# jkflying/opencalibration

Hardware: AMD Instinct MI355X
Metric: images/sec end-to-end (extract+match+relax) on synthetic aerial grid; LM iters/sec (higher is better)
Workload: dtype f32 (extract) + fp4 0/1 bits, f32 accumulate, exact (match) + f64 (RANSAC, relax)

## Files before the change

### opencalibration_amd/csrc/host/extract_features.cpp

```cpp
#include "../env.hpp"
#include "extract_features.hpp"
#include "sort_like_std.hpp"

#include <algorithm>
#include <cmath>
#include <condition_variable>
#include <cstdio>
#include <cstdlib>
#include <cstring>
#include <deque>
#include <limits>
#include <mutex>
#include <thread>

#include <emmintrin.h>
#include <omp.h>

namespace opencalibration_amd
{

namespace
{
struct nn_grid
{
    static constexpr int CAP = 4;
    static constexpr uint32_t EMPTY = 0xffffffffu;
    long gw, gh;
    uint32_t *cells;
    const double *px, *py;
    const uint32_t *home;
    std::vector<uint32_t> overflow;
    nn_grid(double cell, double minx, double miny, double maxx, double maxy, const double *px_, const double *py_, uint32_t n)
        : px(px_), py(py_)
    {
        gw = (long)std::floor((maxx - minx) / cell) + 3;
        gh = (long)std::floor((maxy - miny) / cell) + 3;
        static thread_local std::vector<uint32_t> buf, homes;
        if (buf.size() < (size_t)(gw * gh) * CAP)
            buf.resize((size_t)(gw * gh) * CAP);
        cells = buf.data();
        std::memset(cells, 0xff, (size_t)(gw * gh) * CAP * sizeof(uint32_t));
        homes.resize(n);
        for (uint32_t i = 0; i < n; i++)
            homes[i] = (uint32_t)(((long)((py[i] - miny) / cell) + 1) * gw + (long)((px[i] - minx) / cell) + 1);
        home = homes.data();
    }
    void prefetch(uint32_t i) const
    {
        const uint32_t *c = cells + (size_t)home[i] * CAP;
        __builtin_prefetch(c - (gw + 1) * CAP);
        __builtin_prefetch(c - (gw - 1) * CAP + CAP - 1);
        __builtin_prefetch(c - CAP);
        __builtin_prefetch(c + 2 * CAP - 1);
        __builtin_prefetch(c + (gw - 1) * CAP);
        __builtin_prefetch(c + (gw + 1) * CAP + CAP - 1);
    }
    void add(uint32_t i)
    {
        uint32_t *c = cells + (size_t)home[i] * CAP;
        for (int e = 0; e < CAP; e++)
            if (c[e] == EMPTY)
            {
                c[e] = i;
                return;
            }
        overflow.push_back(i);
    }
    bool any_within(uint32_t i, double scale2, double radius2) const
    {
        const double x = px[i], y = py[i];
        auto close = [&](uint32_t k) {
            const double dx = x - px[k], dy = y - py[k];
            double d = 0;
            d += dx * dx;
            d += dy * dy;
            return !(d * scale2 > radius2);
        };
        const uint32_t *c0 = cells + (size_t)home[i] * CAP;
        const __m128i empty = _mm_set1_epi32(-1);
        for (long yy = -1; yy <= 1; yy++)
        {
            const uint32_t *row = c0 + (yy * gw - 1) * CAP;
            unsigned used = 0;
            for (int q = 0; q < 3; q++)
                used |= (unsigned)(0xf ^ _mm_movemask_ps(_mm_castsi128_ps(
                                             _mm_cmpeq_epi32(_mm_loadu_si128((const __m128i *)(row + 4 * q)), empty))))
                        << (4 * q);
            while (used)
            {
                const int q = __builtin_ctz(used);
                used &= used - 1;
                if (close(row[q]))
                    return true;
            }
        }
        for (uint32_t k : overflow)
            if (close(k))
                return true;
        return false;
    }
};

double g_tail_prof[5];
static double thread_cpu_now()
{
    timespec ts;
    clock_gettime(CLOCK_THREAD_CPUTIME_ID, &ts);
    return (double)ts.tv_sec + 1e-9 * (double)ts.tv_nsec;
}

struct by_response
{
    float response;
    uint32_t index;
};

void suppress_in_order(const double *lx, const double *ly, uint32_t n, double minx, double miny, double maxx, double maxy, double scale,
                       double nms_pixel_radius, std::vector<uint32_t> &sparse, std::vector<uint32_t> &dense)
{
    nn_grid grid(nms_pixel_radius / scale, minx, miny, maxx, maxy, lx, ly, n);
    sparse.reserve(n);
    dense.reserve(n);
    grid.add(0);
    sparse.push_back(0);
    for (uint32_t i = 0; i < n; i++)
    {
        if (i + 12 < n)
            grid.prefetch(i + 12);
        if (!grid.any_within(i, scale * scale, nms_pixel_radius * nms_pixel_radius))
        {
            grid.add(i);
            sparse.push_back(i);
        }
        else
            dense.push_back(i);
    }
}

void extract_tail(const float *k6, const uint64_t *dd, uint32_t n, double scale, extracted_features &out)
{
    static const bool prof = ochip_verbose("extract");
    const double tp0 = prof ? thread_cpu_now() : 0;
    double tp1 = 0, tp2 = 0;
    const double nms_pixel_radius = 8;
    std::vector<uint32_t> order(n);
    {
        static thread_local std::vector<by_response> recs;
        recs.resize(n);
        for (uint32_t i = 0; i < n; i++)
            recs[i] = by_response{k6[6 * (size_t)i + 4], i};
        sort_like_std(recs.data(), recs.data() + n, [](const by_response &a, const by_response &c) -> bool { return a.response > c.response; });
        bool tied = false;
        for (uint32_t i = 0; i < n; i++)
        {
            order[i] = recs[i].index;
            tied = tied || (i && recs[i].response == recs[i - 1].response);
        }
        if (prof && tied)
        {
#pragma omp atomic
            g_tail_prof[4] += 1.0;
        }
    }
    if (prof)
        tp1 = thread_cpu_now();
    out.features.clear();
    out.num_sparse_features = 0;
    if (n == 0)
        return;
    static thread_local std::vector<double> lx, ly;
    lx.resize(n);
    ly.resize(n);
    double minx = std::numeric_limits<double>::infinity(), miny = minx, maxx = -minx, maxy = -minx;
    for (uint32_t i = 0; i < n; i++)
    {
        if (i + 32 < n)
            __builtin_prefetch(k6 + 6 * (size_t)order[i + 32]);
        lx[i] = k6[6 * (size_t)order[i]] / scale;
        ly[i] = k6[6 * (size_t)order[i] + 1] / scale;
        minx = std::min(minx, lx[i]);
        maxx = std::max(maxx, lx[i]);
        miny = std::min(miny, ly[i]);
        maxy = std::max(maxy, ly[i]);
    }
    std::vector<uint32_t> sparse, dense;
    suppress_in_order(lx.data(), ly.data(), n, minx, miny, maxx, maxy, scale, nms_pixel_radius, sparse, dense);
    if (prof)
        tp2 = thread_cpu_now();
    out.num_sparse_features = sparse.size();
    out.features.reserve(sparse.size() + dense.size());
    auto emit = [&](uint32_t i) {
        const uint32_t s = order[i];
        feature_2d p;
        p.location[0] = lx[i];
        p.location[1] = ly[i];
        p.strength = k6[6 * (size_t)s + 4];
        std::memcpy(p.descriptor, dd + 8 * (size_t)s, 64);
        out.features.push_back(p);
    };
    constexpr size_t PREFETCH_AHEAD = 24;
    auto emit_all = [&](const std::vector<uint32_t> &list) {
        const size_t m = list.size();
        for (size_t j = 0; j < m; j++)
        {
            if (j + PREFETCH_AHEAD < m)
            {
                const uint32_t s = order[list[j + PREFETCH_AHEAD]];
                __builtin_prefetch(dd + 8 * (size_t)s);
                __builtin_prefetch(k6 + 6 * (size_t)s + 4);
            }
            emit(list[j]);
        }
    };
    emit_all(sparse);
    emit_all(dense);
    if (prof)
    {
        const double tp3 = thread_cpu_now();
        const double d[4] = {tp1 - tp0, tp2 - tp1, tp3 - tp2, tp3 - tp0};
        for (int i = 0; i < 4; i++)
        {
#pragma omp atomic
            g_tail_prof[i] += d[i];
        }
    }
}

void extract_tail_prepared(const uint8_t *records, const float *response, const uint32_t *slot, uint32_t num_sparse, bool conflict,
                           uint32_t n, double scale, extracted_features &out)
{
    static const bool prof = ochip_verbose("extract");
    const double tp0 = prof ? thread_cpu_now() : 0;
    double tp1 = tp0, tp2 = tp0;
    const double nms_pixel_radius = 8;
    out.features.clear();
    out.num_sparse_features = 0;
    if (n == 0)
        return;
    const feature_2d *R = reinterpret_cast<const feature_2d *>(records);
    if (conflict)
    {
        static thread_local std::vector<by_response> recs;
        recs.resize(n);
        for (uint32_t i = 0; i < n; i++)
            recs[i] = by_response{response[i], i};
        sort_like_std(recs.data(), recs.data() + n, [](const by_response &a, const by_response &c) -> bool { return a.response > c.response; });
        if (prof)
            tp1 = thread_cpu_now();
        static thread_local std::vector<double> lx, ly;
        lx.resize(n);
        ly.resize(n);
        double minx = std::numeric_limits<double>::infinity(), miny = minx, maxx = -minx, maxy = -minx;
        for (uint32_t i = 0; i < n; i++)
        {
            const feature_2d &f = R[slot[recs[i].index]];
            lx[i] = f.location[0];
            ly[i] = f.location[1];
            minx = std::min(minx, lx[i]);
            maxx = std::max(maxx, lx[i]);
            miny = std::min(miny, ly[i]);
            maxy = std::max(maxy, ly[i]);
        }
        std::vector<uint32_t> sparse, dense;
        suppress_in_order(lx.data(), ly.data(), n, minx, miny, maxx, maxy, scale, nms_pixel_radius, sparse, dense);
        if (prof)
            tp2 = thread_cpu_now();
        out.features.reserve((size_t)n + 1);
        for (uint32_t i : sparse)
            out.features.push_back(R[slot[recs[i].index]]);
        out.num_sparse_features = out.features.size();
        for (uint32_t i : dense)
            out.features.push_back(R[slot[recs[i].index]]);
        if (prof)
        {
#pragma omp atomic
            g_tail_prof[4] += 1.0;
        }
    }
    else
    {
        out.features.assign(R, R + (size_t)n + 1);
        out.num_sparse_features = num_sparse;
    }
    if (prof)
    {
        const double tp3 = thread_cpu_now();
        const double d[4] = {tp1 - tp0, tp2 - tp1, tp3 - tp2, tp3 - tp0};
        for (int i = 0; i < 4; i++)
        {
#pragma omp atomic
            g_tail_prof[i] += d[i];
        }
    }
}

struct chunk_buffers
{
    float *kp = nullptr;
    uint64_t *desc = nullptr;
    uint8_t *prepared = nullptr;
    ochip_feature_lists lists{};
    std::vector<uint32_t> counts;
    uint32_t first = 0, n = 0;
};
}

uint32_t extract_chunk_size()
{
    if (const char *e = std::getenv("OCHIP_EXTRACT_CHUNK"))
    {
        const long v = std::atol(e);
        if (v >= 1 && v <= 1024)
            return (uint32_t)v;
    }
    return 100;
}

std::vector<extracted_features> extract_features_batch(ochip_ctx *ctx, const uint8_t *images_bgr, uint32_t n_images,
                                                       int width, int height, uint32_t max_keypoints, std::string *error,
                                                       bool images_on_device)
{
    std::vector<extracted_features> out(n_images);
    const bool ok = extract_features_stream(ctx, images_bgr, n_images, width, height, max_keypoints, images_on_device, 0,
                                            [&](uint32_t first, uint32_t count, extracted_features *f) {
                                                for (uint32_t i = 0; i < count; i++)
                                                    out[first + i] = std::move(f[i]);
                                            },
                                            error);
    if (!ok)
        return {};
    return out;
}

bool extract_features_stream(ochip_ctx *ctx, const uint8_t *images_bgr, uint32_t n_images, int width, int height,
                             uint32_t max_keypoints, bool images_on_device, int host_threads,
                             const std::function<void(uint32_t, uint32_t, extracted_features *)> &on_chunk,
                             std::string *error)
{
    if (n_images == 0)
        return true;
    if (width <= 0 || height <= 0)
    {
        std::vector<extracted_features> empty(n_images);
        on_chunk(0, n_images, empty.data());
        return true;
    }
    const int tail_threads = host_threads > 0 ? host_threads : omp_get_max_threads();
    const int max_length_pixels = 1600;
    const double scale = std::min(1.f, float(max_length_pixels) / (float)std::max(width, height));
    const uint32_t host_chunk = 25;
    const uint32_t chunk = std::min(images_on_device ? extract_chunk_size() : host_chunk, n_images);
    const size_t image_bytes = (size_t)width * height * 3;

    uint32_t n_drivers = images_on_device ? 4 : 5;
    if (const char *e = std::getenv("OCHIP_EXTRACT_STREAMS"))
        n_drivers = (uint32_t)std::max(1L, std::min(5L, std::atol(e)));
    const uint32_t n_chunks = (n_images + chunk - 1) / chunk;
    n_drivers = std::min(n_drivers, n_chunks);
    std::vector<ochip_ctx *> ctxs(n_drivers, ctx);
    for (uint32_t d = 1; d < n_drivers; d++)
        if (ochip_ctx_sibling(ctx, d - 1, &ctxs[d]) != OCHIP_OK)
        {
            if (error)
                *error = std::string("ochip_ctx_sibling: ") + ochip_last_error(ctx);
            return false;
        }
    const bool device_tail = !ochip_test_hook("host_tail");
    const double nms_pixel_radius = 8;
    const bool force_host_nms = ochip_test_hook("host_nms");
    const uint32_t n_bufs = 2 * n_drivers;
    std::vector<chunk_buffers> bufs(n_bufs);
    std::vector<ochip_ctx *> buf_ctx(n_bufs);
    std::string fail;
    auto release = [&]() {
        for (uint32_t i = 0; i < n_bufs; i++)
        {
            chunk_buffers &b = bufs[i];
            if (b.kp)
                ochip_host_free(buf_ctx[i], b.kp);
            if (b.desc)
                ochip_host_free(buf_ctx[i], b.desc);
            if (b.prepared)
                ochip_host_free(buf_ctx[i], b.prepared);
            b.kp = nullptr;
            b.desc = nullptr;
            b.prepared = nullptr;
        }
    };
    for (uint32_t i = 0; i < n_bufs; i++)
    {
        chunk_buffers &b = bufs[i];
        buf_ctx[i] = ctxs[i / 2];
        void *p = nullptr, *q = nullptr;
        if (device_tail)
        {
            const size_t rows = (size_t)chunk * max_keypoints;
            const size_t o_resp = (rows + chunk) * 88, o_slot = o_resp + rows * 4, o_ns = o_slot + rows * 4, o_conf = o_ns + (size_t)chunk * 4;
            const size_t pad = ((size_t)chunk + 15) / 16 * 16;
            const size_t o_sub = o_conf + pad, o_nsub = o_sub + (size_t)chunk * OCHIP_SUBSET_CAP * 4, o_sconf = o_nsub + (size_t)chunk * 4;
            if (ochip_host_alloc(buf_ctx[i], o_sconf + pad, &p) != OCHIP_OK)
            {
                release();
                if (error)
                    *error = std::string("ochip_host_alloc: ") + ochip_last_error(buf_ctx[i]);
                return false;
            }
            b.prepared = (uint8_t *)p;
            b.lists.records = b.prepared;
            b.lists.response = (float *)(b.prepared + o_resp);
            b.lists.slot = (uint32_t *)(b.prepared + o_slot);
            b.lists.num_sparse = (uint32_t *)(b.prepared + o_ns);
            b.lists.conflict = b.prepared + o_conf;
            b.lists.subset = (uint32_t *)(b.prepared + o_sub);
            b.lists.num_subset = (uint32_t *)(b.prepared + o_nsub);
            b.lists.subset_conflict = b.prepared + o_sconf;
            b.lists.subset_spacing = 40.0;
            b.counts.resize(chunk);
            continue;
        }
        if (ochip_host_alloc(buf_ctx[i], (size_t)chunk * max_keypoints * 6 * sizeof(float), &p) != OCHIP_OK ||
            ochip_host_alloc(buf_ctx[i], (size_t)chunk * max_keypoints * 8 * sizeof(uint64_t), &q) != OCHIP_OK)
        {
            if (p)
                ochip_host_free(buf_ctx[i], p);
            release();
            if (error)
                *error = std::string("ochip_host_alloc: ") + ochip_last_error(buf_ctx[i]);
            return false;
        }
        b.kp = (float *)p;
        b.desc = (uint64_t *)q;
        b.counts.resize(chunk);
    }
    double tail_cpu_seconds = 0;
    std::mutex mu;
    std::condition_variable cv;
    std::deque<int> ready;
    std::vector<char> buffer_free(n_bufs, 1);
    uint32_t next_chunk = 0, drivers_done = 0;

    std::vector<double> driver_cpu(n_drivers, 0.0);
    auto driver = [&](uint32_t d) {
        ochip_ctx *dctx = ctxs[d];
        int which = 2 * (int)d;
        const double cpu0 = thread_cpu_now();
        struct at_exit
        {
            double &out, t0;
            ~at_exit() { out = thread_cpu_now() - t0; }
        } record{driver_cpu[d], cpu0};
        for (;;)
        {
            uint32_t c;
            {
                std::unique_lock<std::mutex> lk(mu);
                cv.wait(lk, [&] { return buffer_free[which] != 0; });
                if (!fail.empty() || next_chunk >= n_chunks)
                    break;
                c = next_chunk++;
                buffer_free[which] = 0;
            }
            chunk_buffers &b = bufs[which];
            b.first = c * chunk;
            b.n = std::min(chunk, n_images - b.first);
            int wh[2];
            const uint8_t *src = images_bgr + (size_t)b.first * image_bytes;
            int rc;
            if (device_tail)
                rc = images_on_device ? ochip_akaze_features_dev(dctx, src, b.n, width, height, max_keypoints, nms_pixel_radius,
                                                                 b.counts.data(), &b.lists, wh)
                                      : ochip_akaze_features(dctx, src, b.n, width, height, max_keypoints, nms_pixel_radius,
                                                             b.counts.data(), &b.lists, wh);
            else
                rc = images_on_device ? ochip_akaze_batch_dev(dctx, src, b.n, width, height, max_keypoints, b.kp, b.desc,
                                                              b.counts.data(), wh)
                                      : ochip_akaze_batch(dctx, src, b.n, width, height, max_keypoints, b.kp, b.desc,
                                                          b.counts.data(), wh);
            std::unique_lock<std::mutex> lk(mu);
            if (rc != OCHIP_OK)
            {
                if (fail.empty())
                    fail = std::string("ochip_akaze_batch: ") + ochip_last_error(dctx);
                buffer_free[which] = 1;
                break;
            }
            ready.push_back(which);
            cv.notify_all();
            which = 2 * (int)d + ((which + 1) & 1);
        }
        std::unique_lock<std::mutex> lk(mu);
        drivers_done++;
        cv.notify_all();
    };
    std::vector<std::thread> drivers;
    for (uint32_t d = 0; d < n_drivers; d++)
        drivers.emplace_back(driver, d);

    for (;;)
    {
        int which;
        {
            std::unique_lock<std::mutex> lk(mu);
            cv.wait(lk, [&] { return !ready.empty() || drivers_done == n_drivers; });
            if (ready.empty())
                break;
            which = ready.front();
            ready.pop_front();
        }
        chunk_buffers &b = bufs[which];
        double cpu = 0;
        std::vector<extracted_features> done(b.n);
#pragma omp parallel for schedule(dynamic, 1) reduction(+ : cpu) num_threads(tail_threads)
        for (uint32_t i = 0; i < b.n; i++)
        {
            const double t0 = omp_get_wtime();
            if (device_tail)
            {
                const bool conflict = b.lists.conflict[i] != 0 || force_host_nms;
                extract_tail_prepared(b.lists.records + (size_t)i * ((size_t)max_keypoints + 1) * 88,
                                      b.lists.response + (size_t)i * max_keypoints, b.lists.slot + (size_t)i * max_keypoints,
                                      b.lists.num_sparse[i], conflict, b.counts[i], scale, done[i]);
                if (!conflict && !b.lists.subset_conflict[i] && b.lists.num_subset[i] <= OCHIP_SUBSET_CAP)
                {
                    const uint32_t *sub = b.lists.subset + (size_t)i * OCHIP_SUBSET_CAP;
                    done[i].coarse_subset.assign(sub, sub + b.lists.num_subset[i]);
                    done[i].coarse_spacing = b.lists.subset_spacing;
                }
            }
            else
                extract_tail(b.kp + (size_t)i * max_keypoints * 6, b.desc + (size_t)i * max_keypoints * 8, b.counts[i], scale,
                             done[i]);
            cpu += omp_get_wtime() - t0;
        }
        tail_cpu_seconds += cpu;
        const uint32_t chunk_first = b.first, chunk_n = b.n;
        {
            std::unique_lock<std::mutex> lk(mu);
            buffer_free[which] = 1;
            cv.notify_all();
        }
        on_chunk(chunk_first, chunk_n, done.data());
    }
    for (auto &t : drivers)
        t.join();
    if (ochip_verbose("extract"))
    {
        fprintf(stderr, "[extract] %u images: host tail %.3f thread-seconds of wall time (%.2f ms per image)\n", n_images,
                tail_cpu_seconds, 1e3 * tail_cpu_seconds / n_images);
        double dc = 0;
        for (double v : driver_cpu)
            dc += v;
        fprintf(stderr, "[extract] CPU seconds of the %u device driver threads (launching and waiting): %.3f\n", n_drivers, dc);
        fprintf(stderr, "[extract] cumulative CPU seconds of the tail: ordering %.3f, NMS %.3f, feature records %.3f, total %.3f; images with tied responses %.0f\n",
                g_tail_prof[0], g_tail_prof[1], g_tail_prof[2], g_tail_prof[3], g_tail_prof[4]);
    }
    release();
    if (!fail.empty())
    {
        if (error)
            *error = fail;
        return false;
    }
    return true;
}

}

extern "C" void och_extract_tail_profile(double *out5)
{
    for (int i = 0; i < 5; i++)
        out5[i] = opencalibration_amd::g_tail_prof[i];
}

extern "C" void och_sort_by_response(const float *response, uint32_t n, uint32_t *order_out, int use_std)
{
    using opencalibration_amd::by_response;
    std::vector<by_response> recs(n);
    for (uint32_t i = 0; i < n; i++)
        recs[i] = by_response{response[i], i};
    auto comp = [](const by_response &a, const by_response &c) -> bool { return a.response > c.response; };
    if (use_std)
        std::sort(recs.begin(), recs.end(), comp);
    else
        opencalibration_amd::sort_like_std(recs.data(), recs.data() + n, comp);
    for (uint32_t i = 0; i < n; i++)
        order_out[i] = recs[i].index;
}

extern "C" size_t och_extract_tail(const float *kp6, const uint64_t *desc, uint32_t n, double scale, double *loc, float *strength,
                                   uint64_t *desc_out, uint64_t *num_sparse)
{
    opencalibration_amd::extracted_features out;
    opencalibration_amd::extract_tail(kp6, desc, n, scale, out);
    for (size_t i = 0; i < out.features.size(); i++)
    {
        loc[2 * i] = out.features[i].location[0];
        loc[2 * i + 1] = out.features[i].location[1];
        strength[i] = out.features[i].strength;
        std::memcpy(desc_out + 8 * i, out.features[i].descriptor, 64);
    }
    *num_sparse = out.num_sparse_features;
    return out.features.size();
}

extern "C" size_t och_extract_tail_prepared(const uint8_t *records, const float *response, const uint32_t *slot, uint32_t num_sparse_in,
                                            int conflict, uint32_t n, double scale, double *loc, float *strength, uint64_t *desc_out,
                                            uint64_t *num_sparse)
{
    opencalibration_amd::extracted_features out;
    opencalibration_amd::extract_tail_prepared(records, response, slot, num_sparse_in, conflict != 0, n, scale, out);
    for (size_t i = 0; i < out.features.size(); i++)
    {
        loc[2 * i] = out.features[i].location[0];
        loc[2 * i + 1] = out.features[i].location[1];
        strength[i] = out.features[i].strength;
        std::memcpy(desc_out + 8 * i, out.features[i].descriptor, 64);
    }
    *num_sparse = out.num_sparse_features;
    return out.features.size();
}
```

### opencalibration_amd/csrc/host/extract_features.hpp

```cpp
#pragma once

#include "types.hpp"

#include "../../../include/ochip.h"

#include <functional>
#include <string>

namespace opencalibration_amd
{

struct extracted_features
{
    std::vector<feature_2d> features;
    size_t num_sparse_features = 0;
    std::vector<uint32_t> coarse_subset;
    double coarse_spacing = 0;
};

std::vector<extracted_features> extract_features_batch(ochip_ctx *ctx, const uint8_t *images_bgr, uint32_t n_images,
                                                       int width, int height, uint32_t max_keypoints, std::string *error,
                                                       bool images_on_device = false);

bool extract_features_stream(ochip_ctx *ctx, const uint8_t *images_bgr, uint32_t n_images, int width, int height,
                             uint32_t max_keypoints, bool images_on_device, int host_threads,
                             const std::function<void(uint32_t, uint32_t, extracted_features *)> &on_chunk,
                             std::string *error);

}
```

### opencalibration_amd/csrc/host/load_link.cpp

```cpp
#include "../../../include/oc_host.h"

#include "capi_graph.hpp"
#include "extract_features.hpp"
#include "load_link.hpp"

#include <algorithm>
#include <atomic>
#include <chrono>
#include <condition_variable>
#include <cstdlib>
#include <deque>
#include <mutex>
#include <thread>

#include <omp.h>

using namespace opencalibration_amd;

namespace opencalibration_amd
{

std::vector<owned_pair> pair_owners(const std::vector<NodeLinks> &links)
{
    std::vector<owned_pair> out;
    std::unordered_map<size_t, size_t> link_of;
    for (size_t i = 0; i < links.size(); i++)
        link_of.emplace(links[i].node_id, i);
    for (size_t i = 0; i < links.size(); i++)
        for (size_t m : links[i].link_ids)
        {
            size_t owner = i;
            auto it = link_of.find(m);
            if (it != link_of.end() && it->second > i)
            {
                const auto &back = links[it->second].link_ids;
                if (std::find(back.begin(), back.end(), links[i].node_id) != back.end())
                    owner = it->second;
            }
            out.push_back(owned_pair{owner, LinkStage::link_pair(i, m)});
        }
    return out;
}

namespace
{
std::mutex g_extract_gate_mu;
std::condition_variable g_extract_gate_cv;
bool g_extract_gate_busy = false;
thread_local double g_last_gate_wait = 0;
std::mutex g_lane_mu;
std::condition_variable g_lane_cv;
bool g_lane_busy[2] = {false, false};
struct runner_lane
{
    int lane = -1;
    void acquire()
    {
        std::unique_lock<std::mutex> lk(g_lane_mu);
        g_lane_cv.wait(lk, [] { return !g_lane_busy[0] || !g_lane_busy[1]; });
        lane = g_lane_busy[0] ? 1 : 0;
        g_lane_busy[lane] = true;
    }
    ~runner_lane()
    {
        if (lane < 0)
            return;
        {
            std::lock_guard<std::mutex> lk(g_lane_mu);
            g_lane_busy[lane] = false;
        }
        g_lane_cv.notify_all();
    }
};
struct extract_gate
{
    bool held = false;
    void acquire()
    {
        std::unique_lock<std::mutex> lk(g_extract_gate_mu);
        g_extract_gate_cv.wait(lk, [] { return !g_extract_gate_busy; });
        g_extract_gate_busy = true;
        held = true;
    }
    void release()
    {
        if (!held)
            return;
        {
            std::lock_guard<std::mutex> lk(g_extract_gate_mu);
            g_extract_gate_busy = false;
        }
        g_extract_gate_cv.notify_all();
        held = false;
    }
    ~extract_gate() { release(); }
};
}

bool load_link_stream(och_graph *g, ochip_ctx *ctx, LinkStage &link, const std::vector<size_t> &ids, uint32_t first,
                      uint32_t count, const uint8_t *images_bgr, int width, int height, uint32_t max_keypoints,
                      bool images_on_device, const std::vector<owned_pair> &pairs, double *total_out, double *sparse_out,
                      double *t_extract_done)
{
    using clk = std::chrono::steady_clock;
    runner_lane lane_guard;
    lane_guard.acquire();
    const int lane = lane_guard.lane;
    extract_gate gate;
    const auto t_gate = clk::now();
    const char *gate_env = std::getenv("OCHIP_EXTRACT_GATE");
    if (!(gate_env && gate_env[0] == '0'))
        gate.acquire();
    const auto t_begin = clk::now();
    g_last_gate_wait = std::chrono::duration<double>(t_begin - t_gate).count();
    const auto &links = link.links();
    std::unordered_map<size_t, uint32_t> image_of;
    for (uint32_t b = 0; b < count; b++)
        image_of.emplace(ids[first + b], b);
    constexpr size_t range_len = 125;
    struct range
    {
        std::vector<LinkStage::link_pair> pairs;
        uint32_t waiting;
    };
    size_t owner_lo = links.size(), owner_hi = 0;
    for (const owned_pair &op : pairs)
    {
        owner_lo = std::min(owner_lo, op.owner);
        owner_hi = std::max(owner_hi, op.owner + 1);
    }
    const size_t n_ranges = pairs.empty() ? 0 : (owner_hi - owner_lo + range_len - 1) / range_len;
    std::vector<range> ranges(n_ranges);
    for (const owned_pair &op : pairs)
        ranges[(op.owner - owner_lo) / range_len].pairs.push_back(op.pair);
    std::vector<std::vector<uint32_t>> ranges_of_image(count);
    std::vector<uint32_t> ready_at_once;
    for (size_t k = 0; k < n_ranges; k++)
    {
        range &r = ranges[k];
        std::vector<uint32_t> need;
        for (const auto &lp : r.pairs)
        {
            auto a = image_of.find(links[lp.first].node_id);
            if (a != image_of.end())
                need.push_back(a->second);
            auto it = image_of.find(lp.second);
            if (it != image_of.end())
                need.push_back(it->second);
        }
        std::sort(need.begin(), need.end());
        need.erase(std::unique(need.begin(), need.end()), need.end());
        r.waiting = (uint32_t)need.size();
        for (uint32_t im : need)
            ranges_of_image[im].push_back((uint32_t)k);
        if (need.empty() && !r.pairs.empty())
            ready_at_once.push_back((uint32_t)k);
    }

    const char *renv = std::getenv("OCHIP_LINK_RUNNERS");
    const int n_runners = std::max(1, std::min(8, renv ? std::atoi(renv) : 3));
    const int team = omp_get_max_threads();
    const int tail_threads = std::max(1, team / 2), runner_threads = std::max(1, team / (2 * n_runners) + 1);
    std::mutex mu;
    std::condition_variable cv;
    std::deque<uint32_t> ready(ready_at_once.begin(), ready_at_once.end());
    bool no_more = false;
    std::vector<std::thread> runners;
    for (int r = 0; r < n_runners; r++)
    {
        ochip_ctx *rctx = nullptr;
        if (ochip_ctx_sibling(ctx, (uint32_t)((lane ? 13 : 4) + r), &rctx) != OCHIP_OK)
        {
            g->error = std::string("ochip_ctx_sibling: ") + ochip_last_error(ctx);
            {
                std::lock_guard<std::mutex> lk(mu);
                no_more = true;
                ready.clear();
            }
            cv.notify_all();
            for (auto &t : runners)
                t.join();
            return false;
        }
        runners.emplace_back([&, rctx]() {
            for (;;)
            {
                uint32_t k;
                {
                    std::unique_lock<std::mutex> lk(mu);
                    cv.wait(lk, [&] { return !ready.empty() || no_more; });
                    if (ready.empty())
                        return;
                    k = ready.front();
                    ready.pop_front();
                }
                link.run_pairs(g->graph, ranges[k].pairs, rctx, runner_threads);
            }
        });
    }

    double total = 0, sparse = 0;
    const bool ok = extract_features_stream(
        ctx, images_bgr, count, width, height, max_keypoints, images_on_device, tail_threads,
        [&](uint32_t chunk_first, uint32_t chunk_count, extracted_features *f) {
            std::vector<size_t> chunk_ids(chunk_count);
            for (uint32_t i = 0; i < chunk_count; i++)
            {
                image &img = g->graph.getNode(ids[first + chunk_first + i])->payload;
                total += (double)f[i].features.size();
                sparse += (double)f[i].num_sparse_features;
                img.features = std::move(f[i].features);
                img.num_sparse_features = f[i].num_sparse_features;
                img.coarse_subset = std::move(f[i].coarse_subset);
                img.coarse_spacing = f[i].coarse_spacing;
                chunk_ids[i] = ids[first + chunk_first + i];
            }
            link.prepare_images(g->graph, chunk_ids, tail_threads);
            std::lock_guard<std::mutex> lk(mu);
            for (uint32_t i = 0; i < chunk_count; i++)
                for (uint32_t k : ranges_of_image[chunk_first + i])
                    if (--ranges[k].waiting == 0)
                        ready.push_back(k);
            cv.notify_all();
        },
        &g->error);
    gate.release();
    if (t_extract_done)
        *t_extract_done = std::chrono::duration<double>(clk::now() - t_begin).count();
    {
        std::lock_guard<std::mutex> lk(mu);
        no_more = true;
        if (!ok)
            ready.clear();
    }
    cv.notify_all();
    for (auto &t : runners)
        t.join();
    if (!ok)
        return false;
    if (!link.error.empty())
    {
        g->error = link.error;
        return false;
    }
    if (total_out)
        *total_out = total;
    if (sparse_out)
        *sparse_out = sparse;
    return true;
}

std::vector<size_t> add_survey_nodes(och_graph *g, uint32_t n_images, uint32_t model, const double *positions,
                                     const double *orientations, uint64_t *node_ids_out)
{
    std::vector<size_t> ids(n_images);
    for (uint32_t b = 0; b < n_images; b++)
    {
        image img;
        img.model = g->models[model];
        for (int i = 0; i < 3; i++)
            img.position[i] = positions[3 * (size_t)b + i];
        if (orientations)
            for (int i = 0; i < 4; i++)
                img.orientation[i] = orientations[4 * (size_t)b + i];
        img.path = "image_" + std::to_string(g->graph.size_nodes());
        ids[b] = g->graph.addNode(std::move(img));
        if (node_ids_out)
            node_ids_out[b] = ids[b];
    }
    return ids;
}

}

extern "C" int och_graph_load_link_images(och_graph *g, ochip_ctx *ctx, const uint8_t *images_bgr, uint32_t n_images, int width,
                                          int height, uint32_t max_keypoints, int images_on_device, uint32_t model,
                                          const double *positions, const double *orientations, uint64_t *node_ids_out,
                                          double *totals2, double *link_timers8, double *stage_seconds2)
{
    using clk = std::chrono::steady_clock;
    auto seconds_since = [](clk::time_point t0) { return std::chrono::duration<double>(clk::now() - t0).count(); };
    if (!g || !ctx || (n_images && (!images_bgr || !positions)) || model >= g->models.size())
    {
        if (g)
            g->error = "och_graph_load_link_images: bad argument";
        return -1;
    }
    const auto t_begin = clk::now();
    const std::vector<size_t> ids = add_survey_nodes(g, n_images, model, positions, orientations, node_ids_out);
    g->link = std::make_unique<LinkStage>(ctx);
    LinkStage &link = *g->link;
    link.init(g->graph, ids);
    link.prepare_index(g->graph);
    {
        std::unordered_map<size_t, char> mine;
        for (size_t id : ids)
            mine.emplace(id, 1);
        std::vector<size_t> earlier;
        for (const auto &n : g->graph.nodes())
            if (!mine.count(n.id) && !n.payload.features.empty())
                earlier.push_back(n.id);
        if (!earlier.empty())
            link.prepare_images(g->graph, earlier, omp_get_max_threads());
    }
    double total = 0, sparse = 0, t_extract_done = 0;
    if (!load_link_stream(g, ctx, link, ids, 0, n_images, images_bgr, width, height, max_keypoints, images_on_device != 0,
                          pair_owners(link.links()), &total, &sparse, &t_extract_done))
        return -1;
    const double gate_wait = g_last_gate_wait;
    link.finalize(g->graph);
    if (totals2)
    {
        totals2[0] = total;
        totals2[1] = sparse;
    }
    if (link_timers8)
    {
        const LinkTimers &t = link.timers;
        const double v[8] = {t.link_init,  t.subsample,     t.upload,         t.match_device,
                             t.match_host, t.ransac_device, t.decompose_host, t.link_finalize};
        for (int i = 0; i < 8; i++)
            link_timers8[i] = v[i];
    }
    if (stage_seconds2)
    {
        stage_seconds2[0] = t_extract_done;
        stage_seconds2[1] = seconds_since(t_begin) - gate_wait;
    }
    return 0;
}
```

Measured before the change: 3617.

## Replace global extract gate with per-context gates and optional staggered first chunks

Removes the global mutex that serialized whole extraction calls across concurrent load_link_stream lanes. Each driver now gates only on its own device context, so different lanes can overlap extraction on different contexts. Host buffer allocation and freeing are serialized by a new mutex. An opt-in env flag staggers first-chunk sizes per driver to desynchronize the pipeline stages; the risk is more contention on shared contexts and a changed work-distribution pattern.

Result: no change. 3707, median of 4 (+2.5%).

```diff
diff --git a/opencalibration_amd/csrc/host/extract_features.cpp b/opencalibration_amd/csrc/host/extract_features.cpp
--- a/opencalibration_amd/csrc/host/extract_features.cpp
+++ b/opencalibration_amd/csrc/host/extract_features.cpp
@@ -3,6 +3,7 @@
 #include "sort_like_std.hpp"
 
 #include <algorithm>
+#include <chrono>
 #include <cmath>
 #include <condition_variable>
 #include <cstdio>
@@ -303,6 +304,37 @@
     std::vector<uint32_t> counts;
     uint32_t first = 0, n = 0;
 };
+
+std::mutex g_context_gate_mu;
+std::condition_variable g_context_gate_cv;
+std::vector<ochip_ctx *> g_context_busy;
+std::mutex g_result_buffers_mu;
+struct context_gate
+{
+    ochip_ctx *held = nullptr;
+    bool acquire(ochip_ctx *c)
+    {
+        std::unique_lock<std::mutex> lk(g_context_gate_mu);
+        auto busy = [c] { return std::find(g_context_busy.begin(), g_context_busy.end(), c) != g_context_busy.end(); };
+        const bool waited = busy();
+        g_context_gate_cv.wait(lk, [&] { return !busy(); });
+        g_context_busy.push_back(c);
+        held = c;
+        return waited;
+    }
+    void release()
+    {
+        if (!held)
+            return;
+        {
+            std::lock_guard<std::mutex> lk(g_context_gate_mu);
+            g_context_busy.erase(std::find(g_context_busy.begin(), g_context_busy.end(), held));
+        }
+        g_context_gate_cv.notify_all();
+        held = nullptr;
+    }
+    ~context_gate() { release(); }
+};
 }
 
 uint32_t extract_chunk_size()
@@ -335,8 +367,11 @@
 bool extract_features_stream(ochip_ctx *ctx, const uint8_t *images_bgr, uint32_t n_images, int width, int height,
                              uint32_t max_keypoints, bool images_on_device, int host_threads,
                              const std::function<void(uint32_t, uint32_t, extracted_features *)> &on_chunk,
-                             std::string *error)
-{
+                             std::string *error, extract_sharing *sharing)
+{
+    const auto t_call = std::chrono::steady_clock::now();
+    if (sharing)
+        sharing->gate_wait = 0;
     if (n_images == 0)
         return true;
     if (width <= 0 || height <= 0)
@@ -373,6 +408,7 @@
     std::vector<ochip_ctx *> buf_ctx(n_bufs);
     std::string fail;
     auto release = [&]() {
+        std::lock_guard<std::mutex> pools(g_result_buffers_mu);
         for (uint32_t i = 0; i < n_bufs; i++)
         {
             chunk_buffers &b = bufs[i];
@@ -387,6 +423,10 @@
             b.prepared = nullptr;
         }
     };
+    auto pooled_alloc = [](ochip_ctx *c, size_t bytes, void **out) {
+        std::lock_guard<std::mutex> pools(g_result_buffers_mu);
+        return ochip_host_alloc(c, bytes, out);
+    };
     for (uint32_t i = 0; i < n_bufs; i++)
     {
         chunk_buffers &b = bufs[i];
@@ -398,7 +438,7 @@
             const size_t o_resp = (rows + chunk) * 88, o_slot = o_resp + rows * 4, o_ns = o_slot + rows * 4, o_conf = o_ns + (size_t)chunk * 4;
             const size_t pad = ((size_t)chunk + 15) / 16 * 16;
             const size_t o_sub = o_conf + pad, o_nsub = o_sub + (size_t)chunk * OCHIP_SUBSET_CAP * 4, o_sconf = o_nsub + (size_t)chunk * 4;
-            if (ochip_host_alloc(buf_ctx[i], o_sconf + pad, &p) != OCHIP_OK)
+            if (pooled_alloc(buf_ctx[i], o_sconf + pad, &p) != OCHIP_OK)
             {
                 release();
                 if (error)
@@ -418,11 +458,14 @@
             b.counts.resize(chunk);
             continue;
         }
-        if (ochip_host_alloc(buf_ctx[i], (size_t)chunk * max_keypoints * 6 * sizeof(float), &p) != OCHIP_OK ||
-            ochip_host_alloc(buf_ctx[i], (size_t)chunk * max_keypoints * 8 * sizeof(uint64_t), &q) != OCHIP_OK)
+        if (pooled_alloc(buf_ctx[i], (size_t)chunk * max_keypoints * 6 * sizeof(float), &p) != OCHIP_OK ||
+            pooled_alloc(buf_ctx[i], (size_t)chunk * max_keypoints * 8 * sizeof(uint64_t), &q) != OCHIP_OK)
         {
             if (p)
+            {
+                std::lock_guard<std::mutex> pools(g_result_buffers_mu);
                 ochip_host_free(buf_ctx[i], p);
+            }
             release();
             if (error)
                 *error = std::string("ochip_host_alloc: ") + ochip_last_error(buf_ctx[i]);
@@ -437,7 +480,11 @@
     std::condition_variable cv;
     std::deque<int> ready;
     std::vector<char> buffer_free(n_bufs, 1);
-    uint32_t next_chunk = 0, drivers_done = 0;
+    uint32_t next_image = 0, drivers_done = 0;
+    const char *stagger_env = std::getenv("OCHIP_EXTRACT_STAGGER");
+    const bool stagger = images_on_device && n_chunks > n_drivers && stagger_env && stagger_env[0] != '\0' && stagger_env[0] != '0';
+    const bool gated = sharing && sharing->per_context_gate;
+    bool gate_passed = false;
 
     std::vector<double> driver_cpu(n_drivers, 0.0);
     auto driver = [&](uint32_t d) {
@@ -449,20 +496,28 @@
             double &out, t0;
             ~at_exit() { out = thread_cpu_now() - t0; }
         } record{driver_cpu[d], cpu0};
+        context_gate own;
+        const bool waited = gated && own.acquire(dctx);
+        uint32_t take = stagger && !waited ? std::max(1u, chunk * (d + 1) / n_drivers) : chunk;
         for (;;)
         {
-            uint32_t c;
+            chunk_buffers &b = bufs[which];
             {
                 std::unique_lock<std::mutex> lk(mu);
+                if (gated && !gate_passed)
+                {
+                    gate_passed = true;
+                    sharing->gate_wait = std::chrono::duration<double>(std::chrono::steady_clock::now() - t_call).count();
+                }
                 cv.wait(lk, [&] { return buffer_free[which] != 0; });
-                if (!fail.empty() || next_chunk >= n_chunks)
+                if (!fail.empty() || next_image >= n_images)
                     break;
-                c = next_chunk++;
+                b.first = next_image;
+                b.n = std::min(take, n_images - next_image);
+                next_image += b.n;
                 buffer_free[which] = 0;
             }
-            chunk_buffers &b = bufs[which];
-            b.first = c * chunk;
-            b.n = std::min(chunk, n_images - b.first);
+            take = chunk;
             int wh[2];
             const uint8_t *src = images_bgr + (size_t)b.first * image_bytes;
             int rc;
@@ -488,6 +543,7 @@
             cv.notify_all();
             which = 2 * (int)d + ((which + 1) & 1);
         }
+        own.release();
         std::unique_lock<std::mutex> lk(mu);
         drivers_done++;
         cv.notify_all();
diff --git a/opencalibration_amd/csrc/host/extract_features.hpp b/opencalibration_amd/csrc/host/extract_features.hpp
--- a/opencalibration_amd/csrc/host/extract_features.hpp
+++ b/opencalibration_amd/csrc/host/extract_features.hpp
@@ -22,9 +22,15 @@
                                                        int width, int height, uint32_t max_keypoints, std::string *error,
                                                        bool images_on_device = false);
 
+struct extract_sharing
+{
+    bool per_context_gate = false;
+    double gate_wait = 0;
+};
+
 bool extract_features_stream(ochip_ctx *ctx, const uint8_t *images_bgr, uint32_t n_images, int width, int height,
                              uint32_t max_keypoints, bool images_on_device, int host_threads,
                              const std::function<void(uint32_t, uint32_t, extracted_features *)> &on_chunk,
-                             std::string *error);
+                             std::string *error, extract_sharing *sharing = nullptr);
 
 }
diff --git a/opencalibration_amd/csrc/host/load_link.cpp b/opencalibration_amd/csrc/host/load_link.cpp
--- a/opencalibration_amd/csrc/host/load_link.cpp
+++ b/opencalibration_amd/csrc/host/load_link.cpp
@@ -44,9 +44,6 @@
 
 namespace
 {
-std::mutex g_extract_gate_mu;
-std::condition_variable g_extract_gate_cv;
-bool g_extract_gate_busy = false;
 thread_local double g_last_gate_wait = 0;
 std::mutex g_lane_mu;
 std::condition_variable g_lane_cv;
@@ -72,29 +69,6 @@
         g_lane_cv.notify_all();
     }
 };
-struct extract_gate
-{
-    bool held = false;
-    void acquire()
-    {
-        std::unique_lock<std::mutex> lk(g_extract_gate_mu);
-        g_extract_gate_cv.wait(lk, [] { return !g_extract_gate_busy; });
-        g_extract_gate_busy = true;
-        held = true;
-    }
-    void release()
-    {
-        if (!held)
-            return;
-        {
-            std::lock_guard<std::mutex> lk(g_extract_gate_mu);
-            g_extract_gate_busy = false;
-        }
-        g_extract_gate_cv.notify_all();
-        held = false;
-    }
-    ~extract_gate() { release(); }
-};
 }
 
 bool load_link_stream(och_graph *g, ochip_ctx *ctx, LinkStage &link, const std::vector<size_t> &ids, uint32_t first,
@@ -106,13 +80,11 @@
     runner_lane lane_guard;
     lane_guard.acquire();
     const int lane = lane_guard.lane;
-    extract_gate gate;
     const auto t_gate = clk::now();
     const char *gate_env = std::getenv("OCHIP_EXTRACT_GATE");
-    if (!(gate_env && gate_env[0] == '0'))
-        gate.acquire();
-    const auto t_begin = clk::now();
-    g_last_gate_wait = std::chrono::duration<double>(t_begin - t_gate).count();
+    extract_sharing sharing;
+    sharing.per_context_gate = !(gate_env && gate_env[0] == '0');
+    g_last_gate_wait = 0;
     const auto &links = link.links();
     std::unordered_map<size_t, uint32_t> image_of;
     for (uint32_t b = 0; b < count; b++)
@@ -223,10 +195,10 @@
                         ready.push_back(k);
             cv.notify_all();
         },
-        &g->error);
-    gate.release();
+        &g->error, &sharing);
+    g_last_gate_wait = sharing.gate_wait;
     if (t_extract_done)
-        *t_extract_done = std::chrono::duration<double>(clk::now() - t_begin).count();
+        *t_extract_done = std::chrono::duration<double>(clk::now() - t_gate).count() - sharing.gate_wait;
     {
         std::lock_guard<std::mutex> lk(mu);
         no_more = true;
```
